# rwdavies/QUILT

Hardware: AMD Instinct MI355X
Metric: samples/sec on 2Mb region, K=50k haps, 1x coverage; dosage r2 vs CPU ref (higher is better)
Workload: dtype f64

## Files before the change

quilt_amd/csrc/gibbs.hip:

```cpp
#include "panel.hpp"

#include <chrono>
#include <functional>

#include <algorithm>
#include <cmath>
#include <cstdlib>
#include <map>
#include <memory>

#include "gibbs_dev.hpp"
#include "gibbs_blocks.hpp"

namespace qa {
int gibbs3_waves(int Ksp, int C, int share);
void launch_gibbs3(const void *gibbs_params, hipStream_t st);
void launch_block_rate3(const void *gibbs_params, hipStream_t st);
void launch_block3(const void *gibbs_params, hipStream_t st);
void launch_resample3(const void *gibbs_params, hipStream_t st);
}

namespace {

template <int NE, int NW>
__device__ void forward_full_both(Chain<NE, NW> &ch) {
    const int G = ch.G, Ksp = ch.Ksp;
    Col<NE> a[2], e[2];
    GridStreams<Chain<NE, NW>> gs;
    for (int g = 0; g < G; g++) {
        if ((g & 63) == 0) {
            if (g) gs.store_c(ch);
            gs.load_fwd(ch, g);
        }
        const int j = g & 63;
        ch.ld(e[0], ch.eg[0] + (size_t)g * Ksp);
        ch.ld(e[1], ch.eg[1] + (size_t)g * Ksp);
        const double s0 = rl_f64(gs.t0, j), s1 = rl_f64(gs.t1, j);
#pragma unroll
        for (int h = 0; h < 2; h++) {
#pragma unroll
            for (int i = 0; i < NE; i++) {
                if (g == 0) a[h].v[i] = ch.valid[i] ? ch.prior * e[h].v[i] : 0.0;
                else a[h].v[i] = ch.valid[i] ? e[h].v[i] * (s0 * a[h].v[i] + s1 * ch.prior) : 0.0;
            }
        }
        double sm[2];
        ch.sum_col2(a[0], a[1], sm[0], sm[1]);
        const double cc[2] = {1 / sm[0], 1 / sm[1]};
#pragma unroll
        for (int h = 0; h < 2; h++) {
#pragma unroll
            for (int i = 0; i < NE; i++) a[h].v[i] = a[h].v[i] * cc[h];
            ch.st(a[h], ch.alpha[h] + (size_t)g * Ksp);
        }
        gs.set_c(ch.lane, j, cc[0], cc[1]);
    }
    gs.store_c(ch);
    chain_sync<NW>();
}

template <int NE, int NW, bool FASTER>
__device__ void backward_both(Chain<NE, NW> &ch) {
    const int G = ch.G, Ksp = ch.Ksp;
    const double one_over_K = 1 / (double)ch.Ks;
    Col<NE> b[2], e[2];
    GridStreams<Chain<NE, NW>> gs;
    gs.load_bwd(ch, (G - 1) & ~63);
    {
        const int j = (G - 1) & 63;
        const double cl[2] = {rl_f64(gs.c0, j), rl_f64(gs.c1, j)};
#pragma unroll
        for (int h = 0; h < 2; h++) {
#pragma unroll
            for (int i = 0; i < NE; i++) b[h].v[i] = ch.valid[i] ? cl[h] : 0.0;
            ch.stm(b[h], ch.beta[h] + (size_t)(G - 1) * Ksp);
        }
    }
    if (G >= 2) {
        ch.ldm(e[0], ch.eg[0] + (size_t)(G - 1) * Ksp);
        ch.ldm(e[1], ch.eg[1] + (size_t)(G - 1) * Ksp);
    }
    for (int g = G - 2; g >= 0; --g) {
        if ((g & 63) == 63) gs.load_bwd(ch, g & ~63);
        const int j = g & 63;
        Col<NE> en[2];
        ch.ldm(en[0], ch.eg[0] + (size_t)g * Ksp);
        ch.ldm(en[1], ch.eg[1] + (size_t)g * Ksp);
        const double s0 = rl_f64(gs.t0, j), s1 = rl_f64(gs.t1, j);
        const double cg[2] = {rl_f64(gs.c0, j), rl_f64(gs.c1, j)};
        const bool has = !FASTER || rl_i32(gs.has, j) != 0;
        double x[2] = {0, 0};
#pragma unroll
        for (int h = 0; h < 2; h++) {
#pragma unroll
            for (int i = 0; i < NE; i++) {
                if (has) b[h].v[i] = e[h].v[i] * b[h].v[i];
                if (FASTER) x[h] += b[h].v[i];
                else x[h] += ch.valid[i] ? ch.prior * b[h].v[i] : 0.0;
            }
        }
        ch.template bsum<2>(x);
#pragma unroll
        for (int h = 0; h < 2; h++) {
            const double xx = FASTER ? s1 * x[h] * one_over_K : s1 * x[h];
#pragma unroll
            for (int i = 0; i < NE; i++) b[h].v[i] = ch.valid[i] ? cg[h] * (xx + s0 * b[h].v[i]) : 0.0;
            ch.stm(b[h], ch.beta[h] + (size_t)g * Ksp);
        }
        e[0] = en[0];
        e[1] = en[1];
    }
}

#ifndef QA_LEAN_WAVES
#define QA_LEAN_WAVES 2
#endif
template <int NE, int NW, bool LEAN>
__global__ __launch_bounds__(64 * NW) __attribute__((amdgpu_waves_per_eu(LEAN ? QA_LEAN_WAVES : 1))) void k_gibbs(GibbsParams p) {
    __shared__ double s_red[2 * NW * 4];
    __shared__ double s_e[LEAN ? 2 * NE * 64 * NW : 1];
    const int c = blockIdx.x, t = threadIdx.x;
    using CH = Chain<NE, NW>;
    CH ch(p, c, t, s_red);
    constexpr int NT = CH::NT;
    const int lane = ch.lane;
    const int G = ch.G, Ksp = ch.Ksp, R = ch.R, Ks = ch.Ks;
    const double prior = ch.prior;
    bool (&valid)[NE] = ch.valid;
    const double *runif = p.seed_reads ? nullptr : p.runif_reads + (size_t)p.read_off[c] * p.n_its;
    const uint64_t seed_reads = p.seed_reads ? p.seed_reads[c] : 0, seed_shard = p.seed_shard ? p.seed_shard[c] : 0;
    const int first_read = p.first_read[c];
    const bool init_iteratively = p.init_iteratively && first_read >= 0;

    for (int h = 0; h < 3; h++)
        for (int g = t; g < G; g += NT) ch.cv[h][g] = 0.0;
    for (int r = t; r < R; r += NT) ch.Hc[r] = 0;

    {
        Col<NE> one;
#pragma unroll
        for (int i = 0; i < NE; i++) one.v[i] = 1.0;
        for (int h = 0; h < 2; h++)
            for (int g = 0; g < G; g++) ch.st(one, ch.eg[h] + (size_t)g * Ksp);
    }
    chain_sync<NW>();
    if (!init_iteratively) {
        ReadStreams<CH> rs;
        rs.base = -1;
        int r = 0;
        while (r < R) {
            if ((r & 63) == 0 && rs.base != r) rs.load(ch, r, nullptr, 0);
            const int g = rl_i32(rs.wif, r & 63);
            Col<NE> e[2];
#pragma unroll
            for (int i = 0; i < NE; i++) e[0].v[i] = e[1].v[i] = 1.0;
            while (r < R) {
                if ((r & 63) == 0 && rs.base != r) rs.load(ch, r, nullptr, 0);
                if (rl_i32(rs.wif, r & 63) != g) break;
                Col<NE> er;
                {
                    typename CH::ErPre x;
                    ch.ld_pre(x, r);
                    ch.read_emission(er, x, rl_i32(rs.dn, r & 63));
                }
                const int h = rl_i32(rs.H, r & 63) - 1;
#pragma unroll
                for (int i = 0; i < NE; i++) {
                    if (h == 0) e[0].v[i] *= er.v[i];
                    else e[1].v[i] *= er.v[i];
                }
                r++;
            }
            ch.st(e[0], ch.eg[0] + (size_t)g * Ksp);
            ch.st(e[1], ch.eg[1] + (size_t)g * Ksp);
        }
        forward_full_both(ch);
        backward_both<NE, NW, false>(ch);
    } else {
        Col<NE> one;
#pragma unroll
        for (int i = 0; i < NE; i++) one.v[i] = valid[i] ? 1.0 : 0.0;
        for (int h = 0; h < 2; h++) {
            for (int g = 0; g < G; g++) {
                ch.st(one, ch.alpha[h] + (size_t)g * Ksp);
                ch.st(one, ch.beta[h] + (size_t)g * Ksp);
            }
            for (int g = t; g < G; g += NT) ch.cv[h][g] = 1.0;
        }
        chain_sync<NW>();
        for (int h = 0; h < 2; h++) {
            Col<NE> a;
#pragma unroll
            for (int i = 0; i < NE; i++) a.v[i] = valid[i] ? prior * 1.0 : 0.0;
            const double cc = 1 / ch.sum_col(a);
#pragma unroll
            for (int i = 0; i < NE; i++) a.v[i] = a.v[i] * cc;
            ch.st(a, ch.alpha[h]);
            if (t == 0) ch.cv[h][0] = cc;
        }
    }
    chain_sync<NW>();

    int shard_it = 0;
    int status = 0;
    for (int it = 0; it < p.n_its && status == 0; it++) {
        const bool last_sweep = it == p.n_its - 1;
        const bool steady = !init_iteratively || it >= 2;
        Col<NE> a[2];
        int iRead = 0;
        typename CH::ErPre pre_er;
        if (R > 0) ch.ld_pre(pre_er, 0);
        ReadStreams<CH> rs;
        rs.base = -1;
        GridStreams<CH> gs;
        Col<NE> e[2], bt[2];
        ch.ldm(e[0], ch.eg[0]);
        ch.ldm(e[1], ch.eg[1]);
        ch.ldm(bt[0], ch.beta[0]);
        ch.ldm(bt[1], ch.beta[1]);
        for (int g = 0; g < G; g++) {
            if ((g & 63) == 0) {
                if (g) gs.store_c(ch);
                gs.load_fwd(ch, g);
            }
            const int jg = g & 63;
            const bool has = rl_i32(gs.has, jg) != 0;
            Col<NE> en[LEAN ? 1 : 2], bn[LEAN ? 1 : 2];
            if constexpr (!LEAN) {
                const size_t gn = (size_t)min(g + 1, G - 1) * Ksp;
                ch.ldm(en[0], ch.eg[0] + gn);
                ch.ldm(en[1], ch.eg[1] + gn);
                ch.ldm(bn[0], ch.beta[0] + gn);
                ch.ldm(bn[1], ch.beta[1] + gn);
            }
            double cg[2];
            if (g > 0) {
                const double x = rl_f64(gs.t0, jg), t1 = rl_f64(gs.t1, jg);
                const double one_over_K = 1 / (double)Ks;
                const double c2v[2] = {rl_f64(gs.c0, jg), rl_f64(gs.c1, jg)};
                double sp[2];
                ch.sum_col2(a[0], a[1], sp[0], sp[1]);
#pragma unroll
                for (int h = 0; h < 2; h++) {
                    const double alphaConst = t1 * sp[h];
#pragma unroll
                    for (int i = 0; i < NE; i++) {
                        const double inner = (x * a[h].v[i] + alphaConst * one_over_K);
                        a[h].v[i] = valid[i] ? (has ? e[h].v[i] * inner : inner) : 0.0;
                    }
                }
                double sn[2];
                ch.sum_col2(a[0], a[1], sn[0], sn[1]);
#pragma unroll
                for (int h = 0; h < 2; h++) {
                    const double c2 = c2v[h];
                    double aa = 1 / (c2 * sn[h]);
                    cg[h] = c2 * aa;
                    aa *= c2;
#pragma unroll
                    for (int i = 0; i < NE; i++) a[h].v[i] *= aa;
                }
            } else {
#pragma unroll
                for (int h = 0; h < 2; h++) {
#pragma unroll
                    for (int i = 0; i < NE; i++) a[h].v[i] = valid[i] ? prior * e[h].v[i] : 0.0;
                }
                double sn[2];
                ch.sum_col2(a[0], a[1], sn[0], sn[1]);
#pragma unroll
                for (int h = 0; h < 2; h++) {
                    cg[h] = 1 / sn[h];
#pragma unroll
                    for (int i = 0; i < NE; i++) a[h].v[i] *= cg[h];
                }
            }
            bool changed = false;
            Col<NE> ab[2];
            double pC[2] = {1, 1};
            if (has) {
                double s[2] = {0, 0};
#pragma unroll
                for (int i = 0; i < NE; i++) {
                    ab[0].v[i] = a[0].v[i] * bt[0].v[i];
                    ab[1].v[i] = a[1].v[i] * bt[1].v[i];
                    s[0] += ab[0].v[i];
                    s[1] += ab[1].v[i];
                }
                ch.template bsum<2>(s);
                pC[0] = s[0]; pC[1] = s[1];
                if constexpr (LEAN) {
#pragma unroll
                    for (int h = 0; h < 2; h++) {
#pragma unroll
                        for (int i = 0; i < NE; i++) s_e[(h * NE + i) * NT + t] = e[h].v[i];
                    }
                }
            }
            int h_rC = 0, h_rA1 = 1;
            bool normal = false, ginit = false, pass = false;
            while (iRead < R) {
                if ((iRead & 63) == 0 && rs.base != iRead) {
                    if (rs.base >= 0) rs.store(ch);
                    rs.load(ch, iRead, runif, it);
                    if (!runif) rs.u = stream_uniform(seed_reads, (uint64_t)R * it + iRead + lane);
                }
                const int jr = iRead & 63;
                if (rl_i32(rs.wif, jr) != g) break;
                const int r = iRead;
                const typename CH::ErPre cur_er = pre_er;
                iRead++;
                ch.ld_pre(pre_er, min(iRead, R - 1), (iRead & 63) ? rl_i32(rs.nent, iRead & 63) : 64);
                if (rl_i32(rs.cat1, jr) != 0) continue;
                Col<NE> er, ri;
                const int dn_r = rl_i32(rs.dn, jr);
                if (dn_r >= 0) {
                    ch.ld(er, ch.eMatRead + (size_t)dn_r * Ksp);
#pragma unroll
                    for (int i = 0; i < NE; i++) ri.v[i] = fast_rcp(er.v[i]);
                } else {
                    ch.expand_with_rcp(er, ri, cur_er);
                }
                if (steady) normal = true;
                else if (r < first_read && it == 0) pass = true;
                else if (first_read <= r && it == 0) { pass = false; ginit = true; }
                else if (r < first_read && it == 1) { pass = false; ginit = true; }
                else { ginit = false; normal = true; }
                double pA1[2] = {pC[0], pC[1]};
                if (normal) {
                    h_rC = rl_i32(rs.H, jr) - 1;
                    h_rA1 = 1 - h_rC;
                    double s[2] = {0, 0};
                    double s2[2] = {0, 0};
                    if (h_rC == 0) {
                        asm volatile("" ::: "memory");
#pragma unroll
                        for (int i = 0; i < NE; i++) {
                            double &u0 = (i & 1) ? s2[0] : s[0], &u1 = (i & 1) ? s2[1] : s[1];
                            u0 += ab[0].v[i] * ri.v[i];
                            u1 += ab[1].v[i] * er.v[i];
                        }
                        asm volatile("; current label 0" : "+v"(s[0]), "+v"(s[1]), "+v"(s2[0]), "+v"(s2[1]));
                    } else {
                        asm volatile("" ::: "memory");
#pragma unroll
                        for (int i = 0; i < NE; i++) {
                            double &u0 = (i & 1) ? s2[0] : s[0], &u1 = (i & 1) ? s2[1] : s[1];
                            u0 += ab[1].v[i] * ri.v[i];
                            u1 += ab[0].v[i] * er.v[i];
                        }
                        asm volatile("; current label 1" : "+v"(s[0]), "+v"(s[1]), "+v"(s2[0]), "+v"(s2[1]));
                    }
                    s[0] += s2[0]; s[1] += s2[1];
                    ch.template bsum<2>(s);
                    pA1[h_rC] = s[0];
                    pA1[h_rA1] = s[1];
                } else if (ginit) {
                    h_rC = 0; h_rA1 = 1;
                    double s[2] = {0, 0};
#pragma unroll
                    for (int i = 0; i < NE; i++) {
                        s[0] += ab[0].v[i] * er.v[i];
                        s[1] += ab[1].v[i] * er.v[i];
                    }
                    ch.template bsum<2>(s);
                    pC[0] = s[0];
                    pA1[1] = s[1];
                }
                const double P = pC[0] * pC[1], Q = pA1[0] * pA1[1];
                const double denom = P + Q;
                const double rden = fast_rcp(denom);
                const double norm_pC = P * rden, norm_pA1 = Q * rden;
                const double chance = rl_f64(rs.u, jr);
                const double p0 = (h_rC == 0) ? norm_pC : norm_pA1, p1 = (h_rC == 0) ? norm_pA1 : norm_pC;
                const double cs0 = p0, cs1 = p1 + p0;
                const int h_rN = (chance < cs0) ? 0 : ((chance < cs1) ? 1 : 0);
                if (((h_rN != h_rC) || ginit) && !pass) {
                    changed = true;
                    if (lane == jr) rs.H = h_rN + 1;
                    auto mul_e = [&](int h, const Col<NE> &f) {
                        if constexpr (LEAN) {
#pragma unroll
                            for (int i = 0; i < NE; i++) s_e[(h * NE + i) * NT + t] *= f.v[i];
                        } else {
#pragma unroll
                            for (int i = 0; i < NE; i++) e[h].v[i] *= f.v[i];
                        }
                    };
                    if (normal) {
                        if (h_rC == 0) {
#pragma unroll
                            for (int i = 0; i < NE; i++) { a[0].v[i] *= ri.v[i]; ab[0].v[i] *= ri.v[i]; }
                            mul_e(0, ri);
                        } else {
#pragma unroll
// ... 1621 lines not shown
```

quilt_amd/csrc/gibbs3.hip:

```cpp
#include "gibbs_dev.hpp"

#include <type_traits>

namespace {

template <int NE, int NW, bool LEAN = false>
__global__ __launch_bounds__(64 * NW) __attribute__((amdgpu_waves_per_eu(LEAN ? 2 : NW))) void k_gibbs3(GibbsParams p) {
    __shared__ double s_red[2 * NW * 4];
    __shared__ double s_e[LEAN ? 3 * NE * 64 * NW : 1];
    const int c = blockIdx.x, t = threadIdx.x;
    using CH = Chain<NE, NW>;
    CH ch(p, c, t, s_red);
    constexpr int NT = CH::NT;
    constexpr int NH = 3;
    const int G = ch.G, Ksp = ch.Ksp, R = ch.R, Ks = ch.Ks;
    const double prior = ch.prior;
    bool (&valid)[NE] = ch.valid;
    const double *runif = p.seed_reads ? nullptr : p.runif_reads + (size_t)p.read_off[c] * p.n_its;
    const uint64_t seed_reads = p.seed_reads ? p.seed_reads[c] : 0;
    const int first_read = p.first_read[c];
    const bool init_iteratively = p.init_iteratively && first_read >= 0;
    const double one_over_K = 1 / (double)Ks;

    auto sum3 = [&](const Col<NE> (&x)[NH], double (&s)[NH]) {
// ... 513 lines not shown
    __threadfence_block();
    __syncthreads();
}

__device__ inline int sample3(double p0, double p1, double p2, double u);
__device__ inline int resample_label(int hc, double ff, double u) {
    if (hc >= 1 && hc <= 3) return hc;
    if (hc == 0 || hc == 7) return sample3(0.5, 0.5 - ff * 0.5, ff * 0.5, u);
    if (hc == 4) return sample3(0.5, 0.5 - 0.5 * ff, 0, u);
    if (hc == 5) return sample3(0.5, 0, 0.5 * ff, u);
    return sample3(0, 0.5 - ff * 0.5, ff * 0.5, u);
}
__device__ inline int sample3(double p0, double p1, double p2, double u) {
    double p[3] = {p0, p1, p2};
    int perm[3] = {1, 2, 3};
    const double sum = p[0] + p[1] + p[2];
    for (int i = 0; i < 3; i++) p[i] /= sum;
    for (int i = 1; i < 3; i++) {
        const double v = p[i];
        const int q = perm[i];
        int j = i - 1;
        while (j >= 0 && p[j] < v) { p[j + 1] = p[j]; perm[j + 1] = perm[j]; j--; }
        p[j + 1] = v; perm[j + 1] = q;
    }
    p[1] += p[0];
    if (u <= p[0]) return perm[0];
    if (u <= p[1]) return perm[1];
    return perm[2];
}

__device__ inline double log_p_H_class2(const int (&n)[6], double ff) {
    return 0 + n[0] * log(0.5) + n[1] * log(0.5 - ff * 0.5) + n[2] * log(ff * 0.5) + n[3] * log(1 - ff * 0.5) +
           n[4] * log(1 * 0.5 + ff * 0.5) + n[5] * log(1 * 0.5);
}

template <int NE, int NW>
__global__ __launch_bounds__(64 * NW) void k_block3(GibbsParams p) {
    __shared__ double s_red[2 * NW * 4];
    const int c = blockIdx.x, t = threadIdx.x;
    using CH = Chain<NE, NW>;
    CH ch(p, c, t, s_red);
    constexpr int NT = CH::NT;
    constexpr int NH = 3;
    constexpr int RR[6][3] = {{1, 2, 3}, {1, 3, 2}, {2, 1, 3}, {2, 3, 1}, {3, 1, 2}, {3, 2, 1}};
    constexpr int RX[6][3] = {{1, 2, 3}, {1, 3, 2}, {2, 1, 3}, {3, 1, 2}, {2, 3, 1}, {3, 2, 1}};
    const int G = ch.G, Ksp = ch.Ksp, R = ch.R, Ks = ch.Ks;
    const double prior = ch.prior, one_over_K = 1 / (double)Ks;
    const double ff = p.ff_chain ? rl_f64(p.ff_chain[c], 0) : p.ff;
    bool (&valid)[NE] = ch.valid;
    if (__builtin_amdgcn_readfirstlane(p.status[c]) != 0) return;
    auto uni_d = [](const double *q) { return rl_f64(*q, 0); };
    auto uni_i = [](int v) { return __builtin_amdgcn_readfirstlane(v); };
    const int32_t *where = p.blk_where + (size_t)c * G;
    const int32_t *tab = p.blk_tab + (size_t)c * 4 * G;
    const int n_blocks = uni_i(p.blk_n[c]);
    const double *ru = p.seed_shard ? nullptr : p.runif_shard + ((size_t)p.read_off[c] * p.blk_n_pass + (size_t)p.blk_pass * R) * 2;
    const uint64_t seed = p.seed_shard ? p.seed_shard[c] : 0;
    auto u_block = [&](int i) { return ru ? ru[i] : stream_uniform(seed, (uint64_t)p.blk_pass * 2 * R + i); };
    auto u_draw = [&](int r) { return ru ? ru[R + r] : stream_uniform(seed, (uint64_t)p.blk_pass * 2 * R + R + r); };
    const bool foreign = NW == 2 && p.er_nt == 64;
    int rb_base = -1, rb_wif = 0, rb_H = 0, rb_dn = 0;
    auto rb_get = [&](int r) {
        if (rb_base < 0 || r < rb_base || r >= rb_base + 64) {
            rb_base = r & ~63;
            const int q = rb_base + ch.lane;
            const bool ok = q < R;
            rb_wif = ok ? ch.wif[q] : -1;
            rb_H = ok ? ch.H[q] : 1;
            rb_dn = ok ? ch.dense_of[q] : -1;
        }
        return r - rb_base;
    };
    auto wif_of = [&](int r) { const int j = rb_get(r); return rl_i32(rb_wif, j); };
    auto H_of = [&](int r) { const int j = rb_get(r); return rl_i32(rb_H, j); };
    auto emission_of = [&](Col<NE> &er, int r) {
        const int dn = rl_i32(rb_dn, rb_get(r));
        if (dn >= 0) { ch.ld(er, ch.eMatRead + (size_t)dn * Ksp); return; }
        if (!foreign) {
            typename CH::ErPre x;
            ch.ld_pre(x, r);
            ch.expand(er, x);
            return;
        }
        struct __attribute__((packed, aligned(4))) U3 { uint32_t a, b, c; };
        const U3 q = *reinterpret_cast<const U3 *>(ch.eridx + ((size_t)r * 64 + ch.lane) * 12);
        const uint32_t w4[4] = {q.a, q.b, q.c, 0u};
        const double tv = ch.ertab[(size_t)r * 64 + ch.lane];
        const int lo = __double2loint(tv), hi = __double2hiint(tv);
#pragma unroll
        for (int i = 0; i < NE; i++) {
            uint32_t code = 0;
#pragma unroll
            for (int b = 0; b < 12; b++)
                if (b == ch.wave + 2 * i) code = (w4[b >> 2] >> ((b & 3) * 8)) & 0xffu;
            const int src = (int)code << 2;
            er.v[i] = __hiloint2double(__builtin_amdgcn_ds_bpermute(src, hi), __builtin_amdgcn_ds_bpermute(src, lo));
        }
    };
    auto sum3 = [&](const Col<NE> (&x)[NH], double (&s)[NH]) {
#pragma unroll
        for (int h = 0; h < NH; h++) {
            s[h] = 0;
#pragma unroll
            for (int i = 0; i < NE; i++) s[h] += x[h].v[i];
        }
        ch.template bsum<NH>(s);
    };

    constexpr int EM[6][3] = {{0, 1, 2}, {0, 2, 1}, {1, 0, 2}, {2, 0, 1}, {1, 2, 0}, {2, 1, 0}};
    Col<NE> aS[3][3];
    double inside[3][3];
    double logC_before[3] = {0, 0, 0}, logC_after[3];
    {
        double s[3] = {0, 0, 0};
        for (int g = t; g < G; g += NT)
#pragma unroll
            for (int h = 0; h < 3; h++) s[h] += log(ch.cv[h][g]);
        ch.template bsum<3>(s);
#pragma unroll
        for (int h = 0; h < 3; h++) logC_after[h] = s[h];
    }
#pragma unroll
    for (int h = 0; h < 3; h++)
#pragma unroll
        for (int i = 0; i < 3; i++) inside[h][i] = 0;
    bool ever_changed = false;

    Col<NE> e[NH];
#pragma unroll
    for (int h = 0; h < NH; h++) ch.ld(e[h], ch.eg[h]);
    int where_l = -1;
    double t0_l = 1.0, t1_l = 0.0;
    for (int g = 0; g < G; g++) {
        if ((g & 63) == 0) {
            const int gg = g + ch.lane;
            where_l = gg < G ? where[gg] : -1;
            t0_l = (gg < G && gg > 0) ? ch.tm0(gg - 1) : 1.0;
            t1_l = (gg < G && gg > 0) ? ch.tm1(gg - 1) : 0.0;
        }
        Col<NE> en[NH];
        {
            const size_t gn = (size_t)min(g + 1, G - 1) * Ksp;
#pragma unroll
            for (int h = 0; h < NH; h++) ch.ld(en[h], ch.eg[h] + gn);
        }
        const double t0 = rl_f64(t0_l, g & 63), t1 = rl_f64(t1_l, g & 63);
        double d_of_lane = 1.0;
#pragma unroll
        for (int h = 0; h < 3; h++) {
            Col<NE> nx[NH];
#pragma unroll
            for (int i = 0; i < 3; i++) {
#pragma unroll
                for (int q = 0; q < NE; q++) {
                    if (g == 0) nx[i].v[q] = valid[q] ? prior * e[i].v[q] : 0.0;
                    else nx[i].v[q] = valid[q] ? e[i].v[q] * (t0 * aS[h][i].v[q] + t1 * one_over_K) : 0.0;
                }
            }
            double sm[NH];
            sum3(nx, sm);
#pragma unroll
            for (int i = 0; i < 3; i++) {
                const double d = 1 / sm[i];
                if (ch.lane == 3 * h + i) d_of_lane = d;
#pragma unroll
                for (int q = 0; q < NE; q++) aS[h][i].v[q] = d * nx[i].v[q];
            }
        }
        {
            const double lg = log(d_of_lane);
#pragma unroll
            for (int h = 0; h < 3; h++)
#pragma unroll
                for (int i = 0; i < 3; i++) inside[h][i] += rl_f64(lg, 3 * h + i);
        }
        const int iBlock = rl_i32(where_l, g & 63);
        if (iBlock > -1) {
// ... 269 lines not shown
```

quilt_amd/csrc/gibbs_dev.hpp:

```cpp
#pragma once

#include "panel.hpp"

#include <cstdint>

namespace {

struct GibbsParams {
    const uint8_t *hm;
    const int32_t *B;
    const int32_t *sp_off;
    const int32_t *sp_k;
    const uint32_t *sp_word;
    const double *sigma;
    int Kp, G, T, nMaxDH;
    double ref_error;
    int C;
    int Ks, Ksp, NE;
    const int32_t *which;
    const int32_t *read_off;
    const int32_t *read_ptr;
    const int32_t *base_off;
    const int32_t *u;
    const int32_t *bq;
// ... 72 lines not shown
}
__device__ __forceinline__ double wsum(double v) {
    v += dpp_get<0x111, 0xf>(v);
    v += dpp_get<0x112, 0xf>(v);
    v += dpp_get<0x114, 0xf>(v);
    v += dpp_get<0x118, 0xf>(v);
    v += dpp_get<0x142, 0xa>(v);
    v += dpp_get<0x143, 0xc>(v);
    const int lo = __builtin_amdgcn_readlane(__double2loint(v), 63);
    const int hi = __builtin_amdgcn_readlane(__double2hiint(v), 63);
    return __hiloint2double(hi, lo);
}
__device__ __forceinline__ void wsum2(double &a, double &b) {
    const auto lo = __builtin_amdgcn_permlane32_swap(__double2loint(a), __double2loint(b), false, false);
    const auto hi = __builtin_amdgcn_permlane32_swap(__double2hiint(a), __double2hiint(b), false, false);
    double v = __hiloint2double(hi[0], lo[0]) + __hiloint2double(hi[1], lo[1]);
    v += dpp_get<0x111, 0xf>(v);
    v += dpp_get<0x112, 0xf>(v);
    v += dpp_get<0x114, 0xf>(v);
    v += dpp_get<0x118, 0xf>(v);
    v += dpp_get<0x142, 0xa>(v);
    a = __hiloint2double(__builtin_amdgcn_readlane(__double2hiint(v), 31), __builtin_amdgcn_readlane(__double2loint(v), 31));
    b = __hiloint2double(__builtin_amdgcn_readlane(__double2hiint(v), 63), __builtin_amdgcn_readlane(__double2loint(v), 63));
}
__device__ __forceinline__ double fold32(double a, double b) {
    const auto lo = __builtin_amdgcn_permlane32_swap(__double2loint(a), __double2loint(b), false, false);
    const auto hi = __builtin_amdgcn_permlane32_swap(__double2hiint(a), __double2hiint(b), false, false);
    return __hiloint2double(hi[0], lo[0]) + __hiloint2double(hi[1], lo[1]);
}
__device__ __forceinline__ double fold16_rows(double ab, double cd) {
    const auto lo = __builtin_amdgcn_permlane16_swap(__double2loint(ab), __double2loint(cd), false, false);
    const auto hi = __builtin_amdgcn_permlane16_swap(__double2hiint(ab), __double2hiint(cd), false, false);
    double v = __hiloint2double(hi[0], lo[0]) + __hiloint2double(hi[1], lo[1]);
    v += dpp_get<0x111, 0xf>(v);
    v += dpp_get<0x112, 0xf>(v);
    v += dpp_get<0x114, 0xf>(v);
    v += dpp_get<0x118, 0xf>(v);
    return v;
}
__device__ __forceinline__ double lane_of(double v, int l) {
    return __hiloint2double(__builtin_amdgcn_readlane(__double2hiint(v), l), __builtin_amdgcn_readlane(__double2loint(v), l));
}
__device__ __forceinline__ void wsum3(double &a, double &b, double &c) {
    const double v = fold16_rows(fold32(a, b), fold32(c, c));
    a = lane_of(v, 15); b = lane_of(v, 47); c = lane_of(v, 31);
}
__device__ __forceinline__ void wsum4(double &a, double &b, double &c, double &d) {
    const double v = fold16_rows(fold32(a, b), fold32(c, d));
    a = lane_of(v, 15); b = lane_of(v, 47); c = lane_of(v, 31); d = lane_of(v, 63);
}
__device__ __forceinline__ double wmax(double v) {
#pragma unroll
    for (int o = 32; o > 0; o >>= 1) v = fmax(v, __shfl_xor(v, o, 64));
    return v;
}

__device__ __forceinline__ double stream_uniform(uint64_t seed, uint64_t i) {
    uint64_t z = seed + (i + 1) * 0x9E3779B97F4A7C15ull;
    z = (z ^ (z >> 30)) * 0xBF58476D1CE4E5B9ull;
    z = (z ^ (z >> 27)) * 0x94D049BB133111EBull;
    z = z ^ (z >> 31);
    return (double)(z >> 11) * (1.0 / 9007199254740992.0);
}

__device__ __forceinline__ uint32_t panel_word(const GibbsParams &p, int g, int k, int code) {
    if (code > 0) return (uint32_t)p.B[(size_t)g * p.nMaxDH + (code - 1)];
    int lo = p.sp_off[g], hi = p.sp_off[g + 1] - 1;
    while (lo < hi) {
        int mid = (lo + hi) >> 1;
        if (p.sp_k[mid] < k) lo = mid + 1; else hi = mid;
    }
    return p.sp_word[lo];
}

__device__ __forceinline__ double rl_f64(double v, int j) {
    const int lo = __builtin_amdgcn_readlane(__double2loint(v), j);
    const int hi = __builtin_amdgcn_readlane(__double2hiint(v), j);
    return __hiloint2double(hi, lo);
}
__device__ __forceinline__ int rl_i32(int v, int j) { return __builtin_amdgcn_readlane(v, j); }

constexpr int kReadsPerWave = 32;
constexpr int kMaxPatternBits = 5;
constexpr int padb_of(int ne) { return ne <= 4 ? 4 : ne <= 8 ? 8 : ne <= 12 ? 12 : 16; }

template <int NEALL, int NW>
__global__ __launch_bounds__(64) void k_ematread(GibbsParams p) {
    constexpr int NE = NEALL / NW, PADB = padb_of(NE), NT = 64 * NW;
    const int c = blockIdx.y, lane = threadIdx.x;
    const int R = p.read_off[c + 1] - p.read_off[c];
    const int r0 = blockIdx.x * kReadsPerWave;
    if (r0 >= R) return;
    const int32_t *rp = p.read_ptr + p.read_off[c] + c;
    const int32_t *u = p.u + p.base_off[c], *bq = p.bq + p.base_off[c];
    const int32_t *which = p.which + (size_t)c * p.Ks;
    int kk[NEALL];
#pragma unroll
    for (int i = 0; i < NEALL; i++) {
        const int k = lane + 64 * i;
        kk[i] = (k < p.Ks) ? which[k] : -1;
    }
    int g_prev = -1;
    uint32_t w[NEALL];
    const double e1 = 1 - p.ref_error, e0 = p.ref_error;
    const int nblk = min(kReadsPerWave, R - r0);
    static_assert(kReadsPerWave < 64, "lane l holds the offset of read r0 + l, lane nblk the block's end");
    const int my_s = (lane <= nblk) ? rp[r0 + lane] : 0;
    const int my_dense = (lane < nblk) ? p.dense_of[p.read_off[c] + r0 + lane] : -1;
    const int b_end = rl_i32(my_s, nblk);
    int chunk0 = rl_i32(my_s, 0), c_u = 0, c_b = 0;
    double c_R = 0, c_A = 0;
    auto load_chunk = [&](int base) {
        chunk0 = base;
        const int idx = base + lane;
        const bool ok = idx < b_end;
        c_u = ok ? u[idx] : 0;
        c_b = ok ? bq[idx] : 0;
        const int ab = c_b < 0 ? -c_b : c_b;
        c_R = p.pR_tab[(c_b > 0 ? 256 : 0) + ab];
        c_A = p.pA_tab[(c_b > 0 ? 256 : 0) + ab];
    };
    load_chunk(chunk0);
    for (int r = r0; r < r0 + nblk; r++) {
        double v[NEALL];
        uint32_t pat[NEALL];
#pragma unroll
        for (int i = 0; i < NEALL; i++) { v[i] = 1.0; pat[i] = 0; }
        const int s = rl_i32(my_s, r - r0);
        int J = rl_i32(my_s, r - r0 + 1) - s - 1;
        if (J >= p.Jmax) J = p.Jmax;
        const int dense = rl_i32(my_dense, r - r0);
        int n_inf = 0;
        double tv = 1.0;
        for (int j = 0; j <= J; j++) {
            if (s + j >= chunk0 + 64) load_chunk(s + j);
            const int li = s + j - chunk0;
            const int b = rl_i32(c_b, li);
            int snp = rl_i32(c_u, li);
            if (p.rc_common) {
                const int all_snp = snp;
                snp = p.rc_common[all_snp];
                if (snp < 0) {
                    if (b == 0) continue;
                    const double pR = rl_f64(c_R, li), pA = rl_f64(c_A, li);
                    const double xe1 = e0 * pA + e1 * pR;
                    const bool any = (p.rc_any[(size_t)c * p.rc_words + (all_snp >> 5)] >> (all_snp & 31)) & 1u;
                    if (!any) {
                        if (!p.rescale) {
#pragma unroll
                            for (int i = 0; i < NEALL; i++) v[i] *= xe1;
                            tv *= xe1;
                        }
                        continue;
                    }
                    const double ratio = (e1 * pA + e0 * pR) / xe1;
#pragma unroll
                    for (int i = 0; i < NEALL; i++) {
                        const uint32_t bit = (kk[i] >= 0 && rare_has_alt(p, kk[i], all_snp)) ? 1u : 0u;
                        v[i] *= xe1;
                        if (bit) v[i] *= ratio;
                        pat[i] |= bit << min(n_inf, 7);
                    }
                    tv *= xe1;
                    if ((lane >> min(n_inf, 31)) & 1) tv *= ratio;
                    n_inf++;
                    continue;
                }
            }
            const int g = snp >> 5;
            if (g != g_prev) {
#pragma unroll
                for (int i = 0; i < NEALL; i++) {
                    w[i] = 0;
                    if (kk[i] >= 0) w[i] = panel_word(p, g, kk[i], p.hm[(size_t)g * p.Kp + kk[i]]);
                }
                g_prev = g;
            }
            if (b == 0) continue;
            const double pR = rl_f64(c_R, li), pA = rl_f64(c_A, li);
            const double f1 = (e1 * pA + (1 - e1) * pR), f0 = (e0 * pA + (1 - e0) * pR);
#pragma unroll
            for (int i = 0; i < NEALL; i++) {
                const uint32_t bit = (w[i] >> (snp & 31)) & 1u;
                v[i] *= bit ? f1 : f0;
                pat[i] |= bit << min(n_inf, 7);
            }
            tv *= ((lane >> min(n_inf, 31)) & 1) ? f1 : f0;
            n_inf++;
        }
        bool degenerate = false;
        double d1 = 1.0;
        if (p.rescale) {
            double x = 0;
#pragma unroll
            for (int i = 0; i < NEALL; i++) if (kk[i] >= 0 && v[i] > x) x = v[i];
            x = wmax(x);
            d1 = 1 / x;
            degenerate = isinf(x) || x == 0 || isinf(d1);
            if (degenerate) {
#pragma unroll
                for (int i = 0; i < NEALL; i++) v[i] = 1;
                tv = 1;
            } else {
#pragma unroll
                for (int i = 0; i < NEALL; i++) {
                    v[i] *= d1;
                    if (v[i] < p.inv_maxdiff) v[i] = p.inv_maxdiff;
                }
                tv *= d1;
                if (tv < p.inv_maxdiff) tv = p.inv_maxdiff;
            }
        }
        const double thresh = 1 - 1e-12;
        bool below = false;
#pragma unroll
        for (int i = 0; i < NEALL; i++) if (kk[i] >= 0 && v[i] < thresh) below = true;
        const bool any_below = __any(below);
        if (lane == 0) {
            p.is_cat1[p.read_off[c] + r] = (any_below || p.disable_read_category_usage) ? 0 : 1;
            p.er_nent[p.read_off[c] + r] = (uint8_t)(n_inf <= kMaxPatternBits ? (1 << n_inf) : 64);
        }
        if (dense >= 0) {
            double *out = p.eMatRead + p.eread_off[c] + (size_t)dense * p.Ksp;
#pragma unroll
            for (int i = 0; i < NEALL; i++) out[lane + 64 * i] = (kk[i] >= 0) ? v[i] : 1.0;
        } else {
            p.er_tab[(size_t)(p.read_off[c] + r) * 64 + lane] = (lane < (1 << n_inf) && lane != 63) ? tv : 1.0;
            uint8_t *ix = p.er_idx + p.eridx_off[c] + (size_t)r * NT * PADB;
#pragma unroll
            for (int wv = 0; wv < NW; wv++) {
                uint32_t pk[PADB / 4];
#pragma unroll
                for (int q = 0; q < PADB / 4; q++) pk[q] = 0;
#pragma unroll
                for (int i = 0; i < NE; i++) {
                    const int j = wv + NW * i;
                    const uint32_t code = (kk[j] >= 0 && !degenerate) ? pat[j] : 63u;
                    pk[i >> 2] |= code << ((i & 3) * 8);
                }
                uint32_t *dst = reinterpret_cast<uint32_t *>(ix + (size_t)(lane + 64 * wv) * PADB);
#pragma unroll
                for (int q = 0; q < PADB / 4; q++) dst[q] = pk[q];
            }
        }
    }
}

template <int NE>
struct Col {
    double v[NE];
};

__device__ __forceinline__ __amdgpu_buffer_rsrc_t buf_rsrc(const void *base, uint32_t bytes) {
    return __builtin_amdgcn_make_buffer_rsrc(const_cast<void *>(base), 0, (int)bytes, 0x00020000);
}
__device__ __forceinline__ double buf_ld_f64(__amdgpu_buffer_rsrc_t r, uint32_t byte_off) {
    return __builtin_bit_cast(double, __builtin_amdgcn_raw_buffer_load_b64(r, (int)byte_off, 0, 0));
}
__device__ __forceinline__ void buf_st_f64(__amdgpu_buffer_rsrc_t r, uint32_t byte_off, double v) {
    __builtin_amdgcn_raw_buffer_store_b64(__builtin_bit_cast(__attribute__((__vector_size__(2 * sizeof(unsigned int)))) unsigned int, v), r,
                                          (int)byte_off, 0, 0);
}

template <int NE>
__device__ __forceinline__ void load_col(Col<NE> &c, const double *src, int t, int NT) {
#pragma unroll
    for (int i = 0; i < NE; i++) c.v[i] = src[t + NT * i];
}
template <int NE>
__device__ __forceinline__ void store_col(const Col<NE> &c, double *dst, int t, int NT) {
#pragma unroll
    for (int i = 0; i < NE; i++) dst[t + NT * i] = c.v[i];
}

__device__ __forceinline__ double fast_rcp(double e) {
    double r = __builtin_amdgcn_rcp(e);
    r = __builtin_fma(__builtin_fma(-e, r, 1.0), r, r);
    r = __builtin_fma(__builtin_fma(-e, r, 1.0), r, r);
    return r;
}

template <int NE, int NW>
struct Chain {
    static constexpr int NT = 64 * NW;
    const GibbsParams &p;
    int c, t, lane, wave, R, G, Ks, Ksp;
    double *alpha[3], *beta[3], *eg[3], *cv[3];
    const double *eMatRead;
    const uint8_t *eridx;
    const double *ertab;
    const int32_t *dense_of;
    const int32_t *wif;
    const uint8_t *ghr, *cat1, *nent;
    int32_t *H, *Hc;
    double prior;
    bool valid[NE];
    double *red;
    int par;

    __device__ Chain(const GibbsParams &p_, int c_, int t_, double *red_)
        : p(p_), c(c_), t(t_), lane(t_ & 63), wave(t_ >> 6), red(red_), par(0) {
        G = p.G; Ks = p.Ks; Ksp = p.Ksp;
        R = p.read_off[c + 1] - p.read_off[c];
        const size_t mat = (size_t)G * Ksp;
        for (int h = 0; h < 3; h++) {
            const size_t at = ((size_t)c * p.nH + min(h, p.nH - 1)) * mat;
            alpha[h] = p.alpha + at;
            beta[h] = p.beta + at;
            eg[h] = p.eg + at;
        }
        for (int h = 0; h < 3; h++) cv[h] = p.cvec + ((size_t)c * 3 + h) * G;
        eMatRead = p.eMatRead + p.eread_off[c];
        eridx = p.er_idx + p.eridx_off[c];
        ertab = p.er_tab + (size_t)p.read_off[c] * 64;
        dense_of = p.dense_of + p.read_off[c];
        wif = p.wif + p.read_off[c];
        cat1 = p.is_cat1 + p.read_off[c];
        nent = p.er_nent + p.read_off[c];
        ghr = p.grid_has_read + (size_t)c * G;
        H = p.H + p.read_off[c];
        Hc = p.H_class + p.read_off[c];
        prior = 1.0 / Ks;
#pragma unroll
        for (int i = 0; i < NE; i++) valid[i] = (i < NE - 1) ? true : (t + NT * i) < Ks;
    }
    static constexpr int PADB = padb_of(NE);
    struct ErPre {
        uint32_t w[PADB / 4];
        double tv;
    };
    __device__ __forceinline__ void ld_pre(ErPre &x, int r, int nent = 64) const {
        const uint32_t *src = reinterpret_cast<const uint32_t *>(eridx + ((size_t)r * NT + t) * PADB);
        if constexpr (PADB == 16) {
            const uint4 q = *reinterpret_cast<const uint4 *>(src);
            x.w[0] = q.x; x.w[1] = q.y; x.w[2] = q.z; x.w[3] = q.w;
        } else if constexpr (PADB == 12) {
            struct __attribute__((packed, aligned(4))) U3 { uint32_t a, b, c; };
            const U3 q = *reinterpret_cast<const U3 *>(src);
            x.w[0] = q.a; x.w[1] = q.b; x.w[2] = q.c;
        } else if constexpr (PADB == 8) {
            const uint2 q = *reinterpret_cast<const uint2 *>(src);
            x.w[0] = q.x; x.w[1] = q.y;
        } else {
            x.w[0] = *src;
        }
        const double tv = buf_ld_f64(buf_rsrc(ertab + (size_t)r * 64, (uint32_t)nent * 8), (uint32_t)lane * 8);
        x.tv = lane == 63 ? 1.0 : tv;
    }
    __device__ __forceinline__ void expand(Col<NE> &er, const ErPre &x) const {
        const int lo = __double2loint(x.tv), hi = __double2hiint(x.tv);
#pragma unroll
        for (int i = 0; i < NE; i++) {
            const int src = (int)((x.w[i >> 2] >> ((i & 3) * 8)) & 0xffu) << 2;
            er.v[i] = __hiloint2double(__builtin_amdgcn_ds_bpermute(src, hi), __builtin_amdgcn_ds_bpermute(src, lo));
        }
    }
    __device__ __forceinline__ void expand_with_rcp(Col<NE> &er, Col<NE> &ri, const ErPre &x) const {
        const double tvi = fast_rcp(x.tv);
        const int lo = __double2loint(x.tv), hi = __double2hiint(x.tv);
        const int ilo = __double2loint(tvi), ihi = __double2hiint(tvi);
#pragma unroll
        for (int i = 0; i < NE; i++) {
            const int src = (int)((x.w[i >> 2] >> ((i & 3) * 8)) & 0xffu) << 2;
            er.v[i] = __hiloint2double(__builtin_amdgcn_ds_bpermute(src, hi), __builtin_amdgcn_ds_bpermute(src, lo));
            ri.v[i] = __hiloint2double(__builtin_amdgcn_ds_bpermute(src, ihi), __builtin_amdgcn_ds_bpermute(src, ilo));
        }
    }
    __device__ __forceinline__ void read_emission(Col<NE> &er, const ErPre &x, int dn) const {
        if (dn >= 0) ld(er, eMatRead + (size_t)dn * Ksp);
        else expand(er, x);
    }

    __device__ __forceinline__ double tm0(int g) const { return p.sigma[g]; }
    __device__ __forceinline__ double tm1(int g) const { return p.sigma[p.G - 1 + g]; }

    template <int N>
    __device__ __forceinline__ void bsum(double (&x)[N]) {
        if constexpr (N == 1) x[0] = wsum(x[0]);
        if constexpr (N == 2) wsum2(x[0], x[1]);
        if constexpr (N == 3) wsum3(x[0], x[1], x[2]);
        if constexpr (N == 4) wsum4(x[0], x[1], x[2], x[3]);
        static_assert(N >= 1 && N <= 4, "bsum handles 1..4 values");
        if (NW == 1) return;
        double *buf = red + (size_t)par * NW * 4;
        if (lane == 0) {
#pragma unroll
            for (int q = 0; q < N; q++) buf[wave * 4 + q] = x[q];
        }
        asm volatile("s_waitcnt lgkmcnt(0)" ::: "memory");
        __builtin_amdgcn_s_barrier();
        asm volatile("" ::: "memory");
#pragma unroll
        for (int q = 0; q < N; q++) {
            double s = 0;
#pragma unroll
            for (int w = 0; w < NW; w++) s += buf[w * 4 + q];
            x[q] = s;
        }
        par ^= 1;
    }
    __device__ __forceinline__ double bsum1(double v) {
        double x[1] = {v};
        bsum<1>(x);
        return x[0];
    }
    __device__ __forceinline__ double sum_col(const Col<NE> &c) {
        double s = 0;
#pragma unroll
        for (int i = 0; i < NE; i++) s += c.v[i];
        return bsum1(s);
    }
    __device__ __forceinline__ void sum_col2(const Col<NE> &c0, const Col<NE> &c1, double &s0, double &s1) {
        double x[2] = {0, 0};
#pragma unroll
        for (int i = 0; i < NE; i++) { x[0] += c0.v[i]; x[1] += c1.v[i]; }
        bsum<2>(x);
        s0 = x[0]; s1 = x[1];
    }
    __device__ __forceinline__ void ld(Col<NE> &c, const double *src) const { load_col(c, src, t, NT); }
    __device__ __forceinline__ void st(const Col<NE> &c, double *dst) const { store_col(c, dst, t, NT); }
    __device__ __forceinline__ void ldm(Col<NE> &c, const double *src) const {
        const __amdgpu_buffer_rsrc_t r = buf_rsrc(src, (uint32_t)Ks * 8);
#pragma unroll
        for (int i = 0; i < NE; i++) c.v[i] = buf_ld_f64(r, (uint32_t)(t + NT * i) * 8);
    }
    __device__ __forceinline__ void stm(const Col<NE> &c, double *dst) const {
        const __amdgpu_buffer_rsrc_t r = buf_rsrc(dst, (uint32_t)Ks * 8);
#pragma unroll
        for (int i = 0; i < NE; i++) buf_st_f64(r, (uint32_t)(t + NT * i) * 8, c.v[i]);
    }
};

template <class CH>
struct GridStreams {
    double t0, t1;
    double c0, c1;
    int has;
    int base;
    __device__ void load_fwd(const CH &ch, int b) {
        base = b;
        const int g = b + ch.lane;
        const bool ok = g < ch.G;
        t0 = (ok && g > 0) ? ch.tm0(g - 1) : 1.0;
        t1 = (ok && g > 0) ? ch.tm1(g - 1) : 0.0;
        c0 = ok ? ch.cv[0][g] : 1.0;
        c1 = ok ? ch.cv[1][g] : 1.0;
// ... 87 lines not shown
```

Baseline: 36.97.

## Pack emission pattern codes into 6-bit fields and skip unused emission and alpha stores

Pattern codes per thread are repacked from 8-bit into 6-bit fields, five per word, which shrinks the per-read index buffer. The index fetch now goes through buffer loads with a zero-size range when the next read is unused (cat1 or a dense read), so those fetches are suppressed. The initial fill of grid emissions with ones only touches grid points that have no reads, and the initial forward pass stores alpha only when there are no iterations. Together these cut global memory traffic, but they add bit-extraction cost and rely on later code overwriting alpha and the emissions of grid points that do have reads.

```diff
diff --git a/quilt_amd/csrc/gibbs.hip b/quilt_amd/csrc/gibbs.hip
--- a/quilt_amd/csrc/gibbs.hip
+++ b/quilt_amd/csrc/gibbs.hip
@@ -23,7 +23,7 @@
 namespace {
 
 template <int NE, int NW>
-__device__ void forward_full_both(Chain<NE, NW> &ch) {
+__device__ void forward_full_both(Chain<NE, NW> &ch, bool store_alpha) {
     const int G = ch.G, Ksp = ch.Ksp;
     Col<NE> a[2], e[2];
     GridStreams<Chain<NE, NW>> gs;
@@ -51,7 +51,7 @@
         for (int h = 0; h < 2; h++) {
 #pragma unroll
             for (int i = 0; i < NE; i++) a[h].v[i] = a[h].v[i] * cc[h];
-            ch.st(a[h], ch.alpha[h] + (size_t)g * Ksp);
+            if (store_alpha) ch.st(a[h], ch.alpha[h] + (size_t)g * Ksp);
         }
         gs.set_c(ch.lane, j, cc[0], cc[1]);
     }
@@ -140,8 +140,16 @@
         Col<NE> one;
 #pragma unroll
         for (int i = 0; i < NE; i++) one.v[i] = 1.0;
-        for (int h = 0; h < 2; h++)
-            for (int g = 0; g < G; g++) ch.st(one, ch.eg[h] + (size_t)g * Ksp);
+        for (int g0 = 0; g0 < G; g0 += 64) {
+            const int gg = g0 + lane;
+            const unsigned long long fill = __ballot(gg < G && (init_iteratively || ch.ghr[gg] == 0));
+            const int n = min(64, G - g0);
+            for (int j = 0; j < n; j++) {
+                if (!((fill >> j) & 1ull)) continue;
+                ch.st(one, ch.eg[0] + (size_t)(g0 + j) * Ksp);
+                ch.st(one, ch.eg[1] + (size_t)(g0 + j) * Ksp);
+            }
+        }
     }
     chain_sync<NW>();
     if (!init_iteratively) {
@@ -174,7 +182,7 @@
             ch.st(e[0], ch.eg[0] + (size_t)g * Ksp);
             ch.st(e[1], ch.eg[1] + (size_t)g * Ksp);
         }
-        forward_full_both(ch);
+        forward_full_both(ch, p.n_its < 1);
         backward_both<NE, NW, false>(ch);
     } else {
         Col<NE> one;
@@ -310,7 +318,12 @@
                 const int r = iRead;
                 const typename CH::ErPre cur_er = pre_er;
                 iRead++;
-                ch.ld_pre(pre_er, min(iRead, R - 1), (iRead & 63) ? rl_i32(rs.nent, iRead & 63) : 64);
+                {
+                    const int jn = iRead & 63;
+                    const bool unused = rl_i32(rs.cat1, jn) != 0 || rl_i32(rs.dn, jn) >= 0;
+                    const int nent_n = jn ? (unused ? 0 : rl_i32(rs.nent, jn)) : 64;
+                    ch.ld_pre(pre_er, min(iRead, R - 1), nent_n);
+                }
                 if (rl_i32(rs.cat1, jr) != 0) continue;
                 Col<NE> er, ri;
                 const int dn_r = rl_i32(rs.dn, jr);
diff --git a/quilt_amd/csrc/gibbs3.hip b/quilt_amd/csrc/gibbs3.hip
--- a/quilt_amd/csrc/gibbs3.hip
+++ b/quilt_amd/csrc/gibbs3.hip
@@ -619,17 +619,19 @@
             ch.expand(er, x);
             return;
         }
-        struct __attribute__((packed, aligned(4))) U3 { uint32_t a, b, c; };
-        const U3 q = *reinterpret_cast<const U3 *>(ch.eridx + ((size_t)r * 64 + ch.lane) * 12);
-        const uint32_t w4[4] = {q.a, q.b, q.c, 0u};
+        constexpr int FPADB = padb_of(NW * NE);
+        const uint32_t *src_w = reinterpret_cast<const uint32_t *>(ch.eridx + ((size_t)r * 64 + ch.lane) * FPADB);
+        uint32_t wf[FPADB / 4];
+#pragma unroll
+        for (int q = 0; q < FPADB / 4; q++) wf[q] = src_w[q];
         const double tv = ch.ertab[(size_t)r * 64 + ch.lane];
         const int lo = __double2loint(tv), hi = __double2hiint(tv);
 #pragma unroll
         for (int i = 0; i < NE; i++) {
             uint32_t code = 0;
 #pragma unroll
-            for (int b = 0; b < 12; b++)
-                if (b == ch.wave + 2 * i) code = (w4[b >> 2] >> ((b & 3) * 8)) & 0xffu;
+            for (int b = 0; b < NW * NE; b++)
+                if (b == ch.wave + NW * i) code = (wf[b / kPatPerWord] >> pat_shift(b)) & (uint32_t)kPatPad;
             const int src = (int)code << 2;
             er.v[i] = __hiloint2double(__builtin_amdgcn_ds_bpermute(src, hi), __builtin_amdgcn_ds_bpermute(src, lo));
         }
diff --git a/quilt_amd/csrc/gibbs_dev.hpp b/quilt_amd/csrc/gibbs_dev.hpp
--- a/quilt_amd/csrc/gibbs_dev.hpp
+++ b/quilt_amd/csrc/gibbs_dev.hpp
@@ -178,11 +178,15 @@
 
 constexpr int kReadsPerWave = 32;
 constexpr int kMaxPatternBits = 5;
-constexpr int padb_of(int ne) { return ne <= 4 ? 4 : ne <= 8 ? 8 : ne <= 12 ? 12 : 16; }
+constexpr int kPatFieldBits = 6, kPatPerWord = 5, kPatPad = 63;
+static_assert((1 << kMaxPatternBits) - 1 < kPatPad, "a pattern and the padding value 63 must both fit a 6-bit field and differ");
+constexpr int padb_of(int ne) { return 4 * ((ne + kPatPerWord - 1) / kPatPerWord); }
+__device__ __forceinline__ constexpr uint32_t pat_shift(int i) { return (uint32_t)(kPatFieldBits * (i % kPatPerWord)); }
 
 template <int NEALL, int NW>
 __global__ __launch_bounds__(64) void k_ematread(GibbsParams p) {
     constexpr int NE = NEALL / NW, PADB = padb_of(NE), NT = 64 * NW;
+    static_assert(PADB <= 16, "a thread's pattern pack is fetched with one load of at most four words (20 rows per thread)");
     const int c = blockIdx.y, lane = threadIdx.x;
     const int R = p.read_off[c + 1] - p.read_off[c];
     const int r0 = blockIdx.x * kReadsPerWave;
@@ -329,10 +333,13 @@
 #pragma unroll
                 for (int q = 0; q < PADB / 4; q++) pk[q] = 0;
 #pragma unroll
-                for (int i = 0; i < NE; i++) {
-                    const int j = wv + NW * i;
-                    const uint32_t code = (kk[j] >= 0 && !degenerate) ? pat[j] : 63u;
-                    pk[i >> 2] |= code << ((i & 3) * 8);
+                for (int i = 0; i < kPatPerWord * (PADB / 4); i++) {
+                    uint32_t code = (uint32_t)kPatPad;
+                    if (i < NE) {
+                        const int j = wv + NW * (i < NE ? i : 0);
+                        if (kk[j] >= 0 && !degenerate) code = pat[j];
+                    }
+                    pk[i / kPatPerWord] |= code << pat_shift(i);
                 }
                 uint32_t *dst = reinterpret_cast<uint32_t *>(ix + (size_t)(lane + 64 * wv) * PADB);
 #pragma unroll
@@ -426,28 +433,31 @@
         double tv;
     };
     __device__ __forceinline__ void ld_pre(ErPre &x, int r, int nent = 64) const {
-        const uint32_t *src = reinterpret_cast<const uint32_t *>(eridx + ((size_t)r * NT + t) * PADB);
+        const __amdgpu_buffer_rsrc_t pk = buf_rsrc(eridx + (size_t)r * NT * PADB, nent ? (uint32_t)(NT * PADB) : 0u);
+        const int off = t * PADB;
         if constexpr (PADB == 16) {
-            const uint4 q = *reinterpret_cast<const uint4 *>(src);
-            x.w[0] = q.x; x.w[1] = q.y; x.w[2] = q.z; x.w[3] = q.w;
+            const auto q = __builtin_amdgcn_raw_buffer_load_b128(pk, off, 0, 0);
+            x.w[0] = q[0]; x.w[1] = q[1]; x.w[2] = q[2]; x.w[3] = q[3];
         } else if constexpr (PADB == 12) {
-            struct __attribute__((packed, aligned(4))) U3 { uint32_t a, b, c; };
-            const U3 q = *reinterpret_cast<const U3 *>(src);
-            x.w[0] = q.a; x.w[1] = q.b; x.w[2] = q.c;
+            const auto q = __builtin_amdgcn_raw_buffer_load_b96(pk, off, 0, 0);
+            x.w[0] = q[0]; x.w[1] = q[1]; x.w[2] = q[2];
         } else if constexpr (PADB == 8) {
-            const uint2 q = *reinterpret_cast<const uint2 *>(src);
-            x.w[0] = q.x; x.w[1] = q.y;
+            const auto q = __builtin_amdgcn_raw_buffer_load_b64(pk, off, 0, 0);
+            x.w[0] = q[0]; x.w[1] = q[1];
         } else {
-            x.w[0] = *src;
+            x.w[0] = __builtin_amdgcn_raw_buffer_load_b32(pk, off, 0, 0);
         }
         const double tv = buf_ld_f64(buf_rsrc(ertab + (size_t)r * 64, (uint32_t)nent * 8), (uint32_t)lane * 8);
         x.tv = lane == 63 ? 1.0 : tv;
     }
+    static __device__ __forceinline__ int pat_src(const ErPre &x, int i) {
+        return (int)((x.w[i / kPatPerWord] >> pat_shift(i)) & (uint32_t)kPatPad) << 2;
+    }
     __device__ __forceinline__ void expand(Col<NE> &er, const ErPre &x) const {
         const int lo = __double2loint(x.tv), hi = __double2hiint(x.tv);
 #pragma unroll
         for (int i = 0; i < NE; i++) {
-            const int src = (int)((x.w[i >> 2] >> ((i & 3) * 8)) & 0xffu) << 2;
+            const int src = pat_src(x, i);
             er.v[i] = __hiloint2double(__builtin_amdgcn_ds_bpermute(src, hi), __builtin_amdgcn_ds_bpermute(src, lo));
         }
     }
@@ -457,7 +467,7 @@
         const int ilo = __double2loint(tvi), ihi = __double2hiint(tvi);
 #pragma unroll
         for (int i = 0; i < NE; i++) {
-            const int src = (int)((x.w[i >> 2] >> ((i & 3) * 8)) & 0xffu) << 2;
+            const int src = pat_src(x, i);
             er.v[i] = __hiloint2double(__builtin_amdgcn_ds_bpermute(src, hi), __builtin_amdgcn_ds_bpermute(src, lo));
             ri.v[i] = __hiloint2double(__builtin_amdgcn_ds_bpermute(src, ihi), __builtin_amdgcn_ds_bpermute(src, ilo));
         }
```

Result: no change. 36.66 (-0.8%).
